# trifectatechfoundation/zlib-rs

Hardware: NVIDIA H100
Metric: deflate_level6_raw_input_throughput_silesia_small_tar (higher is better)
Workload: dtype u8

## Files before the change

zlib_rs_b200/csrc/zb_engine.cu:

```cuda
#include <cuda_runtime.h>
#include <stdio.h>
#include <stdlib.h>
#include <string.h>
#include <new>
#include "../../include/zb_engine.h"
#include "zb_kernels.cuh"
#include "zb_engine_internal.h"

namespace zb {

constexpr uint32_t kSlowSub9 = 24576;
constexpr uint32_t kTailTiles = 2;
constexpr uint32_t kTailSub = 512;

thread_local char g_err[256] = "";

static void set_err(const char *what, cudaError_t e)
{
    snprintf(g_err, sizeof g_err, "%s: %s", what, cudaGetErrorString(e));
}

#define CK(call)                                                  \
    do {                                                          \
        cudaError_t e_ = (call);                                  \
        if (e_ != cudaSuccess) { set_err(#call, e_); return ZB_E_CUDA; } \
    } while (0)

__global__ void k_match(JobBufs);
__global__ void k_skip(JobBufs);
__global__ void k_nxt(JobBufs);
__global__ void k_path_tiles(JobBufs);
__global__ void k_path_chain(JobBufs, uint32_t, uint32_t);
__global__ void k_path_groups(JobBufs, uint32_t, uint32_t, uint4 *, uint32_t *);
__global__ void k_path_chain2(JobBufs, uint32_t, uint32_t, const uint4 *, uint32_t *, uint32_t *);
__global__ void k_path_mark(JobBufs, const uint32_t *, const uint32_t *);
__global__ void k_iter_lists(JobBufs, uint32_t *, uint32_t *, uint32_t);
__global__ void k_emit(JobBufs);
__global__ void k_holes(JobBufs, uint32_t);
__global__ void k_holes_cmp(JobBufs, uint32_t, uint32_t);
__global__ void k_tail(JobBufs);
__global__ void k_block_hist(JobBufs, uint32_t *);
__global__ void k_build_blocks(JobBufs, const uint32_t *);
__global__ void k_scan_blocks(JobBufs);
__global__ void k_encode(JobBufs);
__global__ void k_finish(JobBufs, const uint32_t *);
__global__ void k_literal_syms(JobBufs);
__global__ void k_stored(JobBufs);
__global__ void k_links2_std(JobBufs, uint32_t);
__global__ void k_links2_roll(JobBufs, uint32_t);
__global__ void k_links_fix_std(JobBufs);
__global__ void k_links_fix_roll(JobBufs);
__global__ void k_slow(JobBufs);
__global__ void k_rle(JobBufs);
__global__ void k_emit_slow(JobBufs);
__global__ void k_tail_slow(JobBufs);
__global__ void k_serial_low(JobBufs);
__global__ void k_links_dict_ghost(JobBufs, uint32_t *);
__global__ void k_links_dict_ghost_apply(JobBufs, const uint32_t *);
__global__ void k_bgzf_setup(BgzfJob, uint64_t);
__global__ void k_serial_low_members(JobBufs, BgzfJob);
__global__ void k_bgzf_medium(JobBufs, BgzfJob);
__global__ void k_bgzf_slow_steps(JobBufs, BgzfJob);
__global__ void k_bgzf_slow_walk(JobBufs, BgzfJob);
__global__ void k_bgzf_hist(JobBufs, BgzfJob, uint32_t *);
__global__ void k_bgzf_build(JobBufs, BgzfJob, const uint32_t *);
__global__ void k_bgzf_size(JobBufs, BgzfJob);
__global__ void k_bgzf_scan(JobBufs, BgzfJob);
__global__ void k_bgzf_encode(JobBufs, BgzfJob);
__global__ void k_bgzf_frame(JobBufs, BgzfJob);

constexpr uint32_t kMatchSmemBytes = (kWSize + kMatchSub + 512) + (kWSize + kMatchSub) * 2 + ((kWSize + kMatchSub) / 32 + 1) * 4 * 4 + 8192;
constexpr uint32_t kPathSmemBytes = kPathTile * 4 * 3;
constexpr uint32_t kLinks2SmemBytes = 65536 * 2 + kLinkTile * 2 + kLinkTile + 64 + 2048;
constexpr uint32_t kSkipSmemBytes = 2 * kWSize * 2 + 2 * (2 * kWSize / 32) * 4 + 8192 + 64;
constexpr uint32_t kSlowSubMax = 24576;
constexpr uint32_t kSlowSmemBytes = (kWSize + kSlowSubMax + kSlowAhead) * 3;
constexpr uint32_t kChainSmemBytes = kChainChunkTiles * kPathHead * 8;
constexpr uint32_t kChain2MaxSmem = 200 * 1024;
constexpr uint32_t kSerialSmemBytes = (65536 + kWSize) * 2 + 35824 + 16;
constexpr uint32_t kSerialSmemQuick = 65536 * 2 + 65536 + 16;

int Engine::init(int dev)
{
    int n = 0;
    cudaError_t e = cudaGetDeviceCount(&n);
    if (e != cudaSuccess || n == 0) {
        snprintf(g_err, sizeof g_err, "no CUDA device (%s)", e == cudaSuccess ? "count 0" : cudaGetErrorString(e));
        return ZB_E_NODEVICE;
    }
    if (dev < 0 || dev >= n) { snprintf(g_err, sizeof g_err, "device %d out of range", dev); return ZB_E_PARAM; }
    device = dev;
    CK(cudaSetDevice(dev));
    CK(cudaStreamCreateWithFlags(&st, cudaStreamNonBlocking));
    CK(cudaStreamCreateWithFlags(&st2, cudaStreamNonBlocking));
    CK(cudaEventCreateWithFlags(&evf, cudaEventDisableTiming));
    CK(cudaEventCreateWithFlags(&evt, cudaEventDisableTiming));
    for (int i = 0; i < kUpChunks; i++) CK(cudaEventCreateWithFlags(&evc[i], cudaEventDisableTiming));
    CK(cudaEventCreateWithFlags(&evk, cudaEventDisableTiming));
    CK(cudaEventCreate(&ev0));
    CK(cudaEventCreate(&ev1));
    CK(upload_tables());
    CK(cudaFuncSetAttribute(k_match, cudaFuncAttributeMaxDynamicSharedMemorySize, kMatchSmemBytes));
    CK(cudaFuncSetAttribute(k_skip, cudaFuncAttributeMaxDynamicSharedMemorySize, kSkipSmemBytes));
    CK(cudaFuncSetAttribute(k_links2_std, cudaFuncAttributeMaxDynamicSharedMemorySize, kLinks2SmemBytes));
    CK(cudaFuncSetAttribute(k_links2_roll, cudaFuncAttributeMaxDynamicSharedMemorySize, kLinks2SmemBytes));
    CK(cudaFuncSetAttribute(k_slow, cudaFuncAttributeMaxDynamicSharedMemorySize, kSlowSmemBytes));
    CK(cudaFuncSetAttribute(k_path_tiles, cudaFuncAttributeMaxDynamicSharedMemorySize, kPathSmemBytes));
    CK(cudaFuncSetAttribute(k_path_mark, cudaFuncAttributeMaxDynamicSharedMemorySize, kPathSmemBytes));
    CK(cudaFuncSetAttribute(k_path_chain, cudaFuncAttributeMaxDynamicSharedMemorySize, kChainSmemBytes));
    CK(cudaFuncSetAttribute(k_path_groups, cudaFuncAttributeMaxDynamicSharedMemorySize, kChain2MaxSmem));
    CK(cudaFuncSetAttribute(k_path_chain2, cudaFuncAttributeMaxDynamicSharedMemorySize, kChain2MaxSmem));
    CK(cudaFuncSetAttribute(k_serial_low, cudaFuncAttributeMaxDynamicSharedMemorySize, kSerialSmemBytes));
    CK(cudaFuncSetAttribute(k_serial_low_members, cudaFuncAttributeMaxDynamicSharedMemorySize, kSerialSmemBytes));
    CK(cudaMallocHost(&h_info, sizeof(JobInfo)));
    CK(cudaMalloc(&d_info, sizeof(JobInfo)));
    CK(cudaMalloc(&d_check, 16));
    { int rc_ = inflate_init(); if (rc_ != ZB_OK) return rc_; }
    return ZB_OK;
}

Engine::~Engine()
{
    if (device < 0) return;
    cudaSetDevice(device);
    for (auto &b : bufs) if (b.p) cudaFree(b.p);
    if (h_stage) cudaFreeHost(h_stage);
    if (h_info) cudaFreeHost(h_info);
    if (d_info) cudaFree(d_info);
    if (d_check) cudaFree(d_check);
    if (ev0) cudaEventDestroy(ev0);
    if (ev1) cudaEventDestroy(ev1);
    if (evf) cudaEventDestroy(evf);
    if (evt) cudaEventDestroy(evt);
    for (int i = 0; i < kUpChunks; i++) if (evc[i]) cudaEventDestroy(evc[i]);
    if (evk) cudaEventDestroy(evk);
    if (st2) cudaStreamDestroy(st2);
    if (st) cudaStreamDestroy(st);
}

void Engine::pbegin()
{
    if (!profile) return;
    if (!pev0) { cudaEventCreate(&pev0); cudaEventCreate(&pev1); }
    cudaEventRecord(pev0, st);
}

void Engine::pend(int phase, uint32_t nlaunch)
{
    if (!profile) return;
    cudaEventRecord(pev1, st);
    cudaEventSynchronize(pev1);
    float ms = 0;
    cudaEventElapsedTime(&ms, pev0, pev1);
    phase_ms[phase] += ms;
    phase_launches[phase] += nlaunch;
}

int Engine::reserve(int slot, size_t bytes, void **out)
{
    Buf &b = bufs[slot];
    if (b.cap < bytes) {
        if (b.p) { cudaFree(b.p); b.p = nullptr; b.cap = 0; }
        size_t want = bytes + (bytes >> 3) + 4096;
        cudaError_t e = cudaMalloc(&b.p, want);
        if (e != cudaSuccess) { set_err("cudaMalloc", e); return ZB_E_MEM; }
        b.cap = want;
// ... 229 lines not shown
        pend(9, 0);
    }
    CK(cudaMemsetAsync(d_info, 0, sizeof(JobInfo), st));
    CK(cudaMemsetAsync(d_out, 0, out_cap, st));
    if (jb.prime_bits) {
        h_prime = (uint8_t)((flags >> 16) & ((1u << jb.prime_bits) - 1u));
        CK(cudaMemcpyAsync(d_out, &h_prime, 1, cudaMemcpyHostToDevice, st));
    }
    cudaStream_t st_ck = chunked_upload ? st2 : st;
    pbegin();
    if (wrap == 1 || (wrap == 0 && (flags & ZB_FLAG_CHECK_ADLER))) { CK(launch_adler32(d_in + dstart, n_in, 1, d_ck, ck_bytes, d_check, st_ck)); launches += 2; }
    else if (wrap == 2 || (wrap == 0 && (flags & ZB_FLAG_CHECK_CRC))) { CK(launch_crc32(d_in + dstart, n_in, 0, d_ck, ck_bytes, d_check, st_ck)); launches += 2; }
    else CK(cudaMemsetAsync(d_check, 0, 4, st_ck));
    if (chunked_upload) CK(cudaEventRecord(evk, st2));
    pend(8, 2);

    auto links_tiles = [&](bool roll) {
        uint32_t t_done = 0;
        for (uint32_t k = 0; k < (chunked_upload ? up_chunks : 1u); k++) {
            uint32_t t_hi = nmt;
            if (chunked_upload) {
                cudaStreamWaitEvent(st, evc[k], 0);
                if (k + 1 < up_chunks) t_hi = up_len[k] >= 64 ? (uint32_t)((up_len[k] - 64) / kLinkTile) : 0;
            }
            if (t_hi <= t_done) continue;
            if (roll) k_links2_roll<<<t_hi - t_done, 1024, kLinks2SmemBytes, st>>>(jb, t_done);
            else k_links2_std<<<t_hi - t_done, 1024, kLinks2SmemBytes, st>>>(jb, t_done);
            if (k) launches++;
            t_done = t_hi;
        }
        if (chunked_upload) cudaStreamWaitEvent(st, evk, 0);
    };
    uint32_t iters = 0;
    if (level == 0) {
        const uint32_t nb = n_in == 0 ? 1 : (uint32_t)((n_in + 65534) / 65535);
        k_stored<<<nb, 256, 0, st>>>(jb);
        launches++;
        k_finish<<<1, 32, 0, st>>>(jb, d_check);
        launches++;
    } else {
        if (jb.huffman_only) {
            k_literal_syms<<<(uint32_t)(n_in / 256 + 1), 256, 0, st>>>(jb);
            launches++;
        } else if (jb.serial_mode) {
            iters = 1;
            pbegin();
            k_serial_low<<<1, 32, jb.serial_mode == 2 ? kSerialSmemBytes : kSerialSmemQuick, st>>>(jb);
            launches++;
            pend(1, 1);
        } else {
            CK(cudaMemsetAsync(jb.holes, 0, (size_t)nwords * 4, st));
            CK(cudaMemsetAsync(jb.holes_new, 0, (size_t)nwords * 4, st));
            CK(cudaMemsetAsync(jb.tile_dirty, 1, nmt, st));
            CK(cudaMemsetAsync(jb.tile_entry, 0xee, (size_t)npt * 4, st));
            CK(cudaMemsetAsync(jb.M + N, 0, (size_t)kPad * 4, st));
            CK(cudaMemsetAsync(jb.L + N, 0, (size_t)kPad * 2, st));
            pbegin();
            if (jb.slow_mode == 2) {
            } else if (jb.slow_mode && jb.sp.slow) {
                links_tiles(true);
                k_links_fix_roll<<<N / 256 + 1, 256, 0, st>>>(jb);
                launches += 2;
            } else {
                links_tiles(false);
                k_links_fix_std<<<N / 256 + 1, 256, 0, st>>>(jb);
                launches += 2;
// ... 74 lines not shown
                    pbegin();
                    k_path_tiles<<<n_ptiles, 1024, kPathSmemBytes, st>>>(jb);
                    launch_chain(first_ptile);
                    launch_mark(iters == 1 ? npt : 2 * n_ptiles + 16);
                    pend(3, 3);
                    pbegin();
                    k_holes<<<(nlists * kLongPerSub + 255) / 256, 256, 0, st>>>(jb, nlists);
                    k_holes_cmp<<<(nwords + 255) / 256, 256, 0, st>>>(jb, nwords, nmt);
                    pend(4, 2);
                    launches += 7;
                    k_iter_lists<<<1, 1024, 0, st>>>(jb, d_lists, d_lists + nmt + 8, npt);
                    launches++;
                    CK(cudaMemcpyAsync(h_info, d_info, sizeof(JobInfo), cudaMemcpyDeviceToHost, st));
                    CK(cudaStreamSynchronize(st));
                    if (h_info->error) { snprintf(g_err, sizeof g_err, "engine error flags 0x%x (parse)", h_info->error); return ZB_E_INTERNAL; }
                    if (getenv("ZB_DEBUG")) {
                        static unsigned long long last[3];
                        if (iters == 1) memset(last, 0, sizeof last);
                        const double ctas = (double)(h_info->dbg[0] - last[0]) + 1e-9;
                        fprintf(stderr, "iter %u dirty %u: ctas %llu stage %.1f walk %.1f kcyc/cta, holes_changed %u, sub %u first_tile %u chain %u\n",
                                iters, n_dirty, h_info->dbg[0] - last[0], (h_info->dbg[1] - last[1]) / 1e3 / ctas,
                                (h_info->dbg[2] - last[2]) / 1e3 / ctas, h_info->holes_changed, jb.match_sub, first_ptile, chain2 ? 2u : 1u);
                        memcpy(last, h_info->dbg, sizeof last);
                    }
                    if (!h_info->holes_changed) break;
                    n_dirty = h_info->n_dirty;
                    if (iters > N / 257u + 4096u) { snprintf(g_err, sizeof g_err, "hole iteration did not converge"); return ZB_E_INTERNAL; }
                }
            }
            CK(cudaEventRecord(evf, st));
            CK(cudaStreamWaitEvent(st2, evf, 0));
            k_tail<<<1, 32, 0, st2>>>(jb);
            launches++;
            CK(cudaEventRecord(evt, st2));
            if (jb.tail_start > 0) {
                pbegin();
                k_emit<<<(jb.tail_start + 255) / 256, 256, 0, st>>>(jb);
                launches++;
                pend(4, 1);
            }
            pbegin();
            CK(cudaStreamWaitEvent(st, evt, 0));
            pend(5, 1);
            }
        }
        CK(cudaMemcpyAsync(h_info, d_info, sizeof(JobInfo), cudaMemcpyDeviceToHost, st));
        CK(cudaStreamSynchronize(st));
        if (h_info->error) { snprintf(g_err, sizeof g_err, "engine error flags 0x%x (tail)", h_info->error); return ZB_E_INTERNAL; }
        const uint32_t nblocks = h_info->n_blocks;
        if (nblocks == 0 || nblocks > max_blocks) { snprintf(g_err, sizeof g_err, "bad block count %u", nblocks); return ZB_E_INTERNAL; }
        pbegin();
        k_block_hist<<<nblocks, 256, 0, st>>>(jb, d_freq);
        k_build_blocks<<<nblocks, 32, 0, st>>>(jb, d_freq);
        k_scan_blocks<<<1, 256, 0, st>>>(jb);
        pend(6, 3);
        pbegin();
        k_encode<<<nblocks, 1024, 0, st>>>(jb);
        k_finish<<<1, 32, 0, st>>>(jb, d_check);
        pend(7, 2);
        launches += 5;
    }
    CK(cudaMemcpyAsync(h_info, d_info, sizeof(JobInfo), cudaMemcpyDeviceToHost, st));
    CK(cudaStreamSynchronize(st));
    CK(cudaGetLastError());
    if (h_info->error) {
        if (h_info->error & 8u) return ZB_E_BUF;
        snprintf(g_err, sizeof g_err, "engine error flags 0x%x (encode)", h_info->error);
        return ZB_E_INTERNAL;
    }
    const uint64_t out_bytes = h_info->out_bytes;
    if (out_bytes > dst_cap) {
        res->out_bytes = out_bytes;
        return ZB_E_BUF;
    }
    if (d_out != dst) {
        pbegin();
        CK(cudaMemcpyAsync(dst, d_out, out_bytes, dst_dev ? cudaMemcpyDeviceToDevice : cudaMemcpyDeviceToHost, st));
        pend(10, 0);
    }
    CK(cudaEventRecord(ev1, st));
    CK(cudaStreamSynchronize(st));
    float ms = 0;
    CK(cudaEventElapsedTime(&ms, ev0, ev1));
    res->out_bytes = out_bytes;
    res->check = h_info->adler;
    res->data_type = (int32_t)h_info->data_type;
    res->iterations = iters;
    res->n_symbols = h_info->n_syms;
    res->n_blocks = h_info->n_blocks;
    res->gpu_launches = launches;
    res->exact_parity = exact ? 1 : 0;
    res->gpu_ms = ms;
    res->bits_used = (uint32_t)(h_info->total_bits & 7u) ? (uint32_t)(h_info->total_bits & 7u) : 8u;
// ... 337 lines not shown
```

zlib_rs_b200/csrc/zb_engine_internal.h:

```cpp
#pragma once
#include <cuda_runtime.h>
#include <stddef.h>
#include <stdint.h>
#include "../../include/zb_engine.h"
#include "zb_kernels.cuh"

namespace zb {

extern thread_local char g_err[256];
size_t deflate_bound(size_t n);

enum { S_IN, S_L, S_HOLES, S_HOLESN, S_M, S_NXT, S_PEXIT, S_PCNT, S_SYMIDX, S_TENTRY, S_TSYMB, S_TDIRTY, S_SYMS, S_SYMB,
       S_BLOCKS, S_SCRATCH, S_FREQ, S_OUT, S_CK, S_INF0, S_INF1, S_PHEAD, S_SK, S_MARKN, S_LLIST, S_LCNT, S_BMAP, S_HDIFF, S_HCOARSE, S_CSTATE, S_LISTS, S_LR, S_LLAST, S_BBASE, S_MCHG, S_GFN, S_KEYS, S_SHARD,
       S_MEMT, S_MEMC,
       S_BGZF,
       S_COUNT };

struct ShardState {
    int phase = 0;
    JobBufs jb;
    uint32_t off = 0, S = 0, E = 0, total = 0;
    uint32_t bs = 0, npt = 0, O = 0, n = 0, blo = 0, nloc = 0;
    bool is_last = false, tables = false;
    uint4 *gfn = nullptr;
    uint32_t chainG = 0, chain_groups = 0, chain2_smem = 0;
    uint32_t freq_lo[320], freq_hi[320];
    zb_shard_span span;
};

struct Engine {
    static constexpr int kSlots = 41;
    struct Buf { void *p = nullptr; size_t cap = 0; };
    int device = -1;
    cudaStream_t st = nullptr, st2 = nullptr;
    cudaEvent_t evf = nullptr, evt = nullptr;
    cudaEvent_t ev0 = nullptr, ev1 = nullptr;
    static constexpr int kUpChunks = 8;
    cudaEvent_t evk = nullptr;
    cudaEvent_t evc[kUpChunks] = {nullptr};
    Buf bufs[kSlots];
    void *h_stage = nullptr;
    size_t h_stage_cap = 0;
    JobInfo *h_info = nullptr, *d_info = nullptr;
    uint32_t *d_check = nullptr;
    void *d_inf_state = nullptr, *h_inf_state = nullptr;
    uint32_t launches = 0;
    uint8_t h_prime = 0;
    static constexpr int kPhases = 12;
    bool profile = false;
    float phase_ms[kPhases] = {0};
    uint32_t phase_launches[kPhases] = {0};
    cudaEvent_t pev0 = nullptr, pev1 = nullptr;
    void pbegin();
    void pend(int phase, uint32_t nlaunch);

    int init(int dev);
    int inflate_init();
    ~Engine();
    int reserve(int slot, size_t bytes, void **out);
    int stage(size_t bytes);
    int deflate(const void *src, size_t n, bool src_dev, void *dst, size_t dst_cap, bool dst_dev, int level, int strategy,
                int window_bits, uint32_t flags, zb_deflate_result *res, const void *dict = nullptr, size_t dict_len = 0);
    int deflate_bgzf(const void *src, size_t n, bool src_dev, void *dst, size_t dst_cap, bool dst_dev, int level, zb_deflate_result *res);
    int inflate(const void *src, size_t n, bool src_dev, void *dst, size_t dst_cap, bool dst_dev, int window_bits,
                zb_inflate_result *res, uint32_t flags = 0);
    int inflate_stream(const uint8_t *d_src, size_t n, uint8_t *d_dst, size_t dst_cap, int window_bits, uint32_t flags,
                       zb_inflate_result *res);
    int inflate_members(const uint8_t *d_src, size_t n, uint8_t *d_dst, size_t dst_cap, int window_bits, zb_inflate_result *res);
// ... 15 lines not shown
```

zlib_rs_b200/csrc/zb_kernels.cu:

```cuda
#include "zb_kernels.cuh"

namespace zb {

__constant__ HuffTables c_tab;

cudaError_t upload_tables()
{
    HuffTables t;
    init_tables(t);
    return cudaMemcpyToSymbol(c_tab, &t, sizeof t);
}

struct GAcc {
    const uint8_t *data;
    uint32_t N;
    const uint16_t *L;
    const uint32_t *holes;
    const uint32_t *M;
    uint32_t w = kWSize;
    __device__ __forceinline__ uint32_t byte(uint32_t y) const
    {
        while (y >= N) {
            if (y < 2 * w) return 0;
            y -= w;
// ... 1112 lines not shown
        syms[k] = s;
        sb[k] = B;
        k++;
    };
    uint32_t fb;
    if (jb.wsize == kWSize) fb = serial_medium(a, jb.N, p0, ins, 1024u, jb.lp, emit);
    else fb = serial_medium(GAccW{a, jb.wsize}, jb.N, p0, ins, 1024u, jb.lp, emit, DynWin{jb.wsize});
    jb.info->n_syms = n_mid + k;
    jb.info->final_base = fb;
    jb.info->n_blocks = (n_mid + k) / jb.block_syms + 1;
}

__device__ __forceinline__ uint32_t sym_end(const Sym &s) { return s.pos + (s.dist ? (uint32_t)s.lc + 3u : 1u); }

__device__ __forceinline__ void block_hist_body(const Sym *syms, uint32_t begin, uint32_t count, uint32_t *fb)
{
    __shared__ uint32_t lf[kLCodes], df[kDCodes];
    for (uint32_t i = threadIdx.x; i < kLCodes; i += blockDim.x) lf[i] = 0;
    if (threadIdx.x < kDCodes) df[threadIdx.x] = 0;
    __syncthreads();
    for (uint32_t i = threadIdx.x; i < count; i += blockDim.x) {
        const Sym s = syms[begin + i];
        if (s.dist == 0) atomicAdd(&lf[s.lc], 1u);
        else {
            atomicAdd(&lf[257 + c_tab.length_code[s.lc]], 1u);
            atomicAdd(&df[d_code(c_tab, s.dist - 1u)], 1u);
        }
    }
    __syncthreads();
    for (uint32_t i = threadIdx.x; i < kLCodes; i += blockDim.x) fb[i] = lf[i];
    if (threadIdx.x < kDCodes) fb[kLCodes + threadIdx.x] = df[threadIdx.x];
}

__global__ void __launch_bounds__(256) k_block_hist(JobBufs jb, uint32_t *freq )
{
    const uint32_t b = blockIdx.x;
    const uint32_t nsyms = jb.info->n_syms, nblocks = jb.info->n_blocks;
    const uint32_t begin = b * jb.block_syms;
    const uint32_t count = (b + 1 < nblocks) ? jb.block_syms : nsyms - begin;
    block_hist_body(jb.syms, begin, count, freq + b * 320);
    if (threadIdx.x == 0) {
        BlockDesc &bd = jb.blocks[b];
        const bool last = b + 1 == nblocks;
        bd.sym_begin = begin;
        bd.sym_count = count;
        bd.last = last && !jb.not_last;
        const uint32_t start = begin == 0 ? jb.start : sym_end(jb.syms[begin - 1]);
        const uint32_t end = last ? jb.N : sym_end(jb.syms[begin + count - 1]);
        bd.in_start = start;
        bd.in_len = end - start;
        uint32_t Bf;
        if (last) Bf = jb.info->final_base;
        else {
            const uint32_t li = begin + count - 1, n_mid = jb.info->n_mid_syms;
            if (jb.serial_mode) {
                Bf = jb.serial_mode == 2 ? jb.block_base[b] : 0;
            } else if (jb.huffman_only) {
                const uint32_t q = jb.syms[li].pos, w = jb.wsize;
                Bf = q < 2 * w ? 0 : w * (1 + (q - 2 * w) / w);
            } else if (jb.slow_mode == 2) {
                Bf = base_at(jb.syms[li].pos, jb.N, jb.wsize);
            } else if (jb.slow_mode) {
                Bf = base_at(jb.syms[li].pos + 1, jb.N, jb.wsize);
            } else Bf = li < n_mid ? wbase_w(DynWin{jb.wsize}, jb.syms[li].pos) : jb.sym_base[li - n_mid];
        }
        bd.have_window = start >= Bf;
    }
}

__device__ __forceinline__ uint32_t brev_bits(uint32_t code, uint32_t len) { return __brev(code) >> (32u - len); }

template <int KIND>
__device__ __forceinline__ uint32_t xbits_of(uint32_t n) { return KIND == 0 ? (n >= 257 ? extra_lbits(n - 257) : 0u) : KIND == 1 ? extra_dbits(n) : extra_blbits(n); }

template <int KIND>
__device__ int build_tree_warp(TreeScratch &s, TreeState &st, CtData *tree, uint32_t *sh_cnt )
{
    constexpr int elems = KIND == 0 ? kLCodes : KIND == 1 ? kDCodes : kBlCodes;
    constexpr int max_length = KIND == 2 ? kMaxBlBits : kMaxBits;
    const uint32_t lane = threadIdx.x & 31;
    int heap_len = 0, max_code = -1;
    for (int b0 = 0; b0 < elems; b0 += 32) {
        const int n = b0 + (int)lane;
        const bool nz = n < elems && tree[n].fc != 0;
        const uint32_t m = __ballot_sync(0xffffffffu, nz);
        if (nz) { s.heap[heap_len + 1 + __popc(m & ((1u << lane) - 1u))] = (uint32_t)n; s.depth[n] = 0; }
        else if (n < elems) tree[n].dl = 0;
        heap_len += __popc(m);
        if (m) max_code = b0 + 31 - __clz(m);
    }
    __syncwarp();
    if (heap_len < 2) {
        if (lane == 0) {
            while (heap_len < 2) {
                const int node = max_code < 2 ? ++max_code : 0;
                s.heap[++heap_len] = (uint32_t)node;
                tree[node].fc = 1;
// ... 217 lines not shown
            o.put((uint32_t)(blcodes - 4), 4);
            for (int r = 0; r < blcodes; r++) o.put(s.bltree[bl_order(r)].dl, 3);
            send_tree_fast(o, s.bltree, s.ltree, lcodes - 1);
            send_tree_fast(o, s.bltree, s.dtree, dcodes - 1);
            b.hdr_bits = o.nbits;
            b.body_bits = 3 + st.opt_len - o.nbits;
        }
        for (int n = (int)lane; n < kLCodes; n += 32) { b.lcode[n] = n <= lmax ? s.ltree[n].fc : 0; b.llen[n] = n <= lmax ? (uint8_t)s.ltree[n].dl : 0; }
        if (lane < (uint32_t)kDCodes) { b.dcode[lane] = (int)lane <= dmax ? s.dtree[lane].fc : 0; b.dlen[lane] = (int)lane <= dmax ? (uint8_t)s.dtree[lane].dl : 0; }
    }
    __syncwarp();
}

__device__ __forceinline__ void build_blocks_body(BlockDesc *gbd, const uint32_t *fb, bool quick, bool first, bool last_piece,
                                                  bool final_block, bool strategy_fixed)
{
    __shared__ TreeScratch s;
    __shared__ BlockDesc bd;
    __shared__ uint32_t fr[320];
    __shared__ uint32_t sh_cnt[16];
    __shared__ TreeState sh_st;
    for (uint32_t i = threadIdx.x; i < 320; i += 32) fr[i] = fb[i];
    for (uint32_t i = threadIdx.x; i < sizeof(BlockDesc) / 4; i += 32)
        reinterpret_cast<uint32_t *>(&bd)[i] = reinterpret_cast<const uint32_t *>(gbd)[i];
    __syncwarp();
    if (quick) {
        if (threadIdx.x == 0) build_quick_piece(c_tab, bd, fr, fr + kLCodes, first, last_piece, final_block);
    } else build_block_warp(s, bd, fr, fr + kLCodes, bd.have_window != 0, strategy_fixed, sh_cnt, &sh_st);
    __syncwarp();
    for (uint32_t i = threadIdx.x; i < sizeof(BlockDesc) / 4; i += 32)
        reinterpret_cast<uint32_t *>(gbd)[i] = reinterpret_cast<const uint32_t *>(&bd)[i];
}

__global__ void __launch_bounds__(32) k_build_blocks(JobBufs jb, const uint32_t *freq)
{
    const uint32_t b = blockIdx.x;
    if (b >= jb.info->n_blocks) return;
    build_blocks_body(&jb.blocks[b], freq + b * 320, jb.serial_mode == 1, b == 0, b + 1 == jb.info->n_blocks, jb.not_last == 0,
                      jb.strategy_fixed != 0);
}

__device__ __forceinline__ void or_bits(uint32_t *out32, uint64_t pos, uint64_t val, uint32_t n)
{
    if (n == 0) return;
    const uint64_t w = pos >> 5;
    const uint32_t sh = (uint32_t)(pos & 31);
    atomicOr(&out32[w], (uint32_t)(val << sh));
    if (sh + n > 32) {
        atomicOr(&out32[w + 1], (uint32_t)(val >> (32 - sh)));
        if (sh + n > 64) atomicOr(&out32[w + 2], (uint32_t)(val >> (64 - sh)));
    }
}

constexpr uint32_t kScanChunk = 1024;
__global__ void __launch_bounds__(256) k_scan_blocks(JobBufs jb)
{
    __shared__ uint64_t s_bits[kScanChunk];
    __shared__ uint64_t s_base[kScanChunk];
    __shared__ uint64_t s_bit;
    const uint32_t nb = jb.info->n_blocks;
    if (threadIdx.x == 0) s_bit = 8ull * jb.hdr_len + jb.prime_bits;
    for (uint32_t c0 = 0; c0 < nb; c0 += kScanChunk) {
        const uint32_t nc = min(kScanChunk, nb - c0);
        for (uint32_t i = threadIdx.x; i < nc; i += blockDim.x) {
            const BlockDesc &bd = jb.blocks[c0 + i];
            s_bits[i] = bd.type == 0 ? (1ull << 63) | (uint16_t)bd.in_len : (uint64_t)bd.hdr_bits + bd.body_bits;
        }
        __syncthreads();
        if (threadIdx.x == 0) {
            uint64_t bit = s_bit;
            for (uint32_t i = 0; i < nc; i++) {
                s_base[i] = bit;
                const uint64_t v = s_bits[i];
                bit = (v >> 63) ? ((bit + 3 + 7) & ~7ull) + 32 + 8ull * (v & 0xffffu) : bit + v;
            }
            s_bit = bit;
        }
        __syncthreads();
        for (uint32_t i = threadIdx.x; i < nc; i += blockDim.x) jb.blocks[c0 + i].bit_base = s_base[i];
        __syncthreads();
    }
    if (threadIdx.x != 0) return;
    uint64_t bit = s_bit;
    if (jb.not_last && jb.end_mode == 0) {
        const uint64_t p = (bit + 3 + 7) & ~7ull;
        jb.info->marker_byte = p >> 3;
        bit = p + 32;
    } else if (jb.not_last && jb.end_mode == 1) {
        or_bits(reinterpret_cast<uint32_t *>(jb.out), bit, 2u, 10);
        bit += 10;
    }
    jb.info->total_bits = bit;
    const uint64_t bytes = (jb.not_last && jb.end_mode ? (bit >> 3) : ((bit + 7) >> 3)) + (jb.wrap == 1 ? 4 : jb.wrap == 2 ? 8 : 0);
    jb.info->out_bytes = bytes;
    jb.info->data_type = jb.blocks[0].sym_count ? jb.blocks[0].data_type : 2u;
    if (bytes > jb.out_cap) { atomicOr(&jb.info->error, 8u); return; }
    if (jb.wrap == 1) {
        const uint32_t lf = (jb.huffman_only || jb.strategy_fixed || jb.level < 2) ? 0 : jb.level < 6 ? 1 : jb.level == 6 ? 2 : 3;
        uint32_t h = ((8u + (jb.cinfo << 4)) << 8) | (lf << 6);
        h += 31 - (h % 31);
        jb.out[0] = (uint8_t)(h >> 8);
        jb.out[1] = (uint8_t)h;
    } else if (jb.wrap == 2) {
        const uint8_t g[10] = {31, 139, 8, 0, 0, 0, 0, 0, (uint8_t)jb.xfl, 3};
        for (int i = 0; i < 10; i++) jb.out[i] = g[i];
    }
}

__device__ __forceinline__ void encode_body(const BlockDesc &bd, const Sym *syms, const uint8_t *in, uint8_t *out, uint32_t *error)
{
    __shared__ HuffTables st;
    __shared__ uint16_t s_lcode[kLCodes], s_dcode[kDCodes];
    __shared__ uint8_t s_llen[kLCodes], s_dlen[kDCodes];
    __shared__ uint64_t warp_sum[32];
    uint32_t *out32 = reinterpret_cast<uint32_t *>(out);
// ... 58 lines not shown
            lens[j] = (uint8_t)n;
            mybits += n;
        }
        uint64_t incl = mybits;
#pragma unroll
        for (int o = 1; o < 32; o <<= 1) {
            const uint64_t t = __shfl_up_sync(0xffffffffu, incl, o);
            if ((int)lane >= o) incl += t;
        }
        if (lane == 31) warp_sum[warp] = incl;
        __syncthreads();
        if (warp == 0) {
            uint64_t ws = warp_sum[lane];
#pragma unroll
            for (int o = 1; o < 32; o <<= 1) {
                const uint64_t t = __shfl_up_sync(0xffffffffu, ws, o);
                if ((int)lane >= o) ws += t;
            }
            warp_sum[lane] = ws;
        }
        __syncthreads();
        uint64_t pos = bd.bit_base + bd.hdr_bits + round_bits + (incl - mybits) + (warp ? warp_sum[warp - 1] : 0);
#pragma unroll
        for (uint32_t j = 0; j < kSymsPerThread; j++) {
            or_bits(out32, pos, vals[j], lens[j]);
            pos += lens[j];
        }
        round_bits += warp_sum[31];
        __syncthreads();
    }
    if (tid == blockDim.x - 1 && round_bits != bd.body_bits) atomicOr(error, 16u);
}

__global__ void __launch_bounds__(1024) k_encode(JobBufs jb)
{
    if (jb.info->error) return;
    encode_body(jb.blocks[blockIdx.x], jb.syms, jb.in, jb.out, &jb.info->error);
}

__global__ void __launch_bounds__(256) k_bgzf_hist(JobBufs jb, BgzfJob bj, uint32_t *freq)
{
    const uint32_t b = blockIdx.x, m = b / kBgzfMaxBlocks, k = b % kBgzfMaxBlocks;
    const JobInfo &mi = bj.minfo[m];
    const uint32_t nsyms = mi.n_syms, nblocks = mi.n_blocks;
    if (k >= nblocks) return;
    const uint32_t base = m * kBgzfStride, len = bj.mlen[m];
    const Sym *syms = jb.syms + base;
    const uint32_t begin = k * jb.block_syms;
    const uint32_t count = k + 1 < nblocks ? jb.block_syms : nsyms - begin;
    block_hist_body(syms, begin, count, freq + (size_t)b * 320);
    if (threadIdx.x == 0) {
        BlockDesc &bd = jb.blocks[b];
        const bool last = k + 1 == nblocks;
        bd.sym_begin = base + begin;
        bd.sym_count = count;
        bd.last = last;
        const uint32_t start = begin == 0 ? 0 : sym_end(syms[begin - 1]);
        const uint32_t end = last ? len : sym_end(syms[begin + count - 1]);
        bd.in_start = base + start;
        bd.in_len = end - start;
        uint32_t Bf;
        if (last) Bf = mi.final_base;
        else if (jb.slow_mode) Bf = base_at(syms[begin + count - 1].pos + 1, len, jb.wsize);
        else Bf = jb.block_base[b];
        bd.have_window = start >= Bf;
    }
}

__global__ void __launch_bounds__(32) k_bgzf_build(JobBufs jb, BgzfJob bj, const uint32_t *freq)
{
// ... 106 lines not shown
```

zlib_rs_b200/csrc/zb_shard.cu:

```cuda
#include <stdio.h>
#include <string.h>
#include "zb_kernels.cuh"
#include "zb_engine_internal.h"
#include "zb_shard.h"

namespace zb {

__global__ void k_slow(JobBufs);
__global__ void k_links2_std(JobBufs, uint32_t);
__global__ void k_links2_roll(JobBufs, uint32_t);
__global__ void k_links_fix_std(JobBufs);
__global__ void k_links_fix_roll(JobBufs);
__global__ void k_path_tiles(JobBufs);
__global__ void k_path_chain(JobBufs, uint32_t, uint32_t);
__global__ void k_path_groups(JobBufs, uint32_t, uint32_t, uint4 *, uint32_t *);
__global__ void k_path_chain2(JobBufs, uint32_t, uint32_t, const uint4 *, uint32_t *, uint32_t *);
__global__ void k_path_mark(JobBufs, const uint32_t *, const uint32_t *);
__global__ void k_emit_slow(JobBufs);
__global__ void k_tail_slow(JobBufs);
__global__ void k_build_blocks(JobBufs, const uint32_t *);
__global__ void k_scan_blocks(JobBufs);
__global__ void k_encode(JobBufs);

static __constant__ HuffTables s_tab;

constexpr uint32_t kLinks2Smem = 65536 * 2 + kLinkTile * 2 + kLinkTile + 64 + 2048;
constexpr uint32_t kPathSmem = kPathTile * 4 * 3;
constexpr uint32_t kChainSmem = kChainChunkTiles * kPathHead * 8;
constexpr uint32_t kChain2Max = 200 * 1024;

__global__ void __launch_bounds__(128) k_shard_entry(JobBufs jb, uint32_t S, uint32_t E, uint2 *out)
{
    const uint32_t c = blockIdx.x * blockDim.x + threadIdx.x;
    if (c >= kShardCand) return;
    const uint32_t te = jb.info->tail_entry;
    uint32_t spec_total = jb.info->n_mid_syms, spec_exit = te;
    if (te < E) { const uint32_t v = jb.nxt[te]; spec_total += (v >> 16) & 0xffu; spec_exit = te + (v & 0xffffu); }
    uint32_t p = S + c, cnt = 0, steps = 0;
    while (p < E) {
        const uint32_t idx = jb.symidx[p];
        if (idx) {
            const uint32_t k = jb.tile_symbase[p / kPathTile] + idx - 1;
            out[c] = make_uint2(spec_exit, cnt + spec_total - k);
            return;
        }
        const uint32_t v = jb.nxt[p];
        if ((v & 0xffffu) == 0 || ++steps > E) { atomicOr(&jb.info->error, 1u); return; }
        cnt += (v >> 16) & 0xffu;
        p += v & 0xffffu;
    }
    out[c] = make_uint2(p, cnt);
}

__global__ void __launch_bounds__(256) k_shard_hist(JobBufs jb, uint32_t *freq, ShardLoc *loc, uint32_t O, uint32_t n, uint32_t blo,
                                                    uint32_t bs)
// ... 286 lines not shown
    if (nl > shard.nloc) {
        const ShardLoc e{ns, 0, 0, 0, 0, 0, {0, 0}};
        SCK(cudaMemcpyAsync(d_loc + shard.nloc, &e, sizeof e, cudaMemcpyHostToDevice, st));
        SCK(cudaMemsetAsync(d_freq + (size_t)shard.nloc * 320, 0, 320 * 4, st));
        if (shard.nloc) memset(shard.freq_hi, 0, sizeof shard.freq_hi);
        else { memset(shard.freq_lo, 0, sizeof shard.freq_lo); memset(shard.freq_hi, 0, sizeof shard.freq_hi); }
        shard.nloc = nl;
        shard.blo = lo;
    }
    const uint32_t nloc = shard.nloc;
    if (!nloc) { shard.phase = 3; shard.span = *span; return ZB_OK; }
    uint32_t holds = 0;
    static thread_local BlockDesc hb;
    static thread_local ShardBlock m;
    for (int k = 0; k < 2; k++) {
        const uint32_t j = k == 0 ? 0 : nloc - 1, b = shard.blo + j;
        if (shard_merge(all, n, pl, b, bs, shard.total, m) != 0) return shard_param("edge records do not add up");
        SCK(cudaMemcpyAsync(&hb, jb.blocks + j, sizeof hb, cudaMemcpyDeviceToHost, st));
        SCK(cudaStreamSynchronize(st));
        hb.sym_count = m.nsyms;
        hb.in_start = m.in_start >= off ? m.in_start - off : 0u;
        hb.in_len = m.in_end - m.in_start;
        hb.last = b == pl.fin;
        hb.have_window = m.in_start >= m.flush_base;
        SCK(cudaMemcpyAsync(jb.blocks + j, &hb, sizeof hb, cudaMemcpyHostToDevice, st));
        SCK(cudaMemcpyAsync(d_freq + (size_t)j * 320, m.freq, 320 * 4, cudaMemcpyHostToDevice, st));
        SCK(cudaStreamSynchronize(st));
        holds |= (shard_holds_first(O, ns, shard.is_last, pl, b, bs) ? 1u : 0u) << (2 * k);
        holds |= (shard_holds_last(O, ns, shard.is_last, pl, b, bs) ? 2u : 0u) << (2 * k);
    }
    SCK(cudaMemcpyAsync(d_xloc, shard.freq_lo, 320 * 4, cudaMemcpyHostToDevice, st));
    SCK(cudaMemcpyAsync(d_xloc + 320, shard.freq_hi, 320 * 4, cudaMemcpyHostToDevice, st));
    SCK(cudaMemcpyAsync(&d_info->n_blocks, &nloc, 4, cudaMemcpyHostToDevice, st));
    k_build_blocks<<<nloc, 32, 0, st>>>(jb, d_freq);
    k_shard_piece<<<1, 256, 0, st>>>(jb, d_freq, d_xloc, d_loc, nloc, holds, d_span);
    SCK(cudaMemcpyAsync(span, d_span, sizeof *span, cudaMemcpyDeviceToHost, st));
    SCK(cudaMemcpyAsync(h_info, d_info, sizeof(JobInfo), cudaMemcpyDeviceToHost, st));
    SCK(cudaStreamSynchronize(st));
    SCK(cudaGetLastError());
    if (h_info->error) { snprintf(g_err, sizeof g_err, "engine error flags 0x%x (shard size)", h_info->error); return ZB_E_INTERNAL; }
    shard.span = *span;
    shard.phase = 3;
    return ZB_OK;
}

int Engine::shard_encode(uint64_t bit_offset, void *dst, size_t cap, bool dst_dev, uint64_t *bytes)
{
    if (shard.phase != 3) { shard.phase = 0; return shard_param("zb_shard_encode needs zb_shard_size first"); }
    if (!bytes) { shard.phase = 0; return shard_param("null argument"); }
    JobBufs &jb = shard.jb;
    const uint32_t prime = (uint32_t)(bit_offset & 7u);
    const uint64_t end = shard_span_end(shard.span, prime), need = (end + 7) >> 3;
    *bytes = need;
    if (cap < need || (!dst && need)) return ZB_E_BUF;
    shard.phase = 0;
    if (!need) return ZB_OK;
    SCK(cudaSetDevice(device));
    if (!shard.nloc) {
        if (dst_dev) SCK(cudaMemset(dst, 0, need)); else memset(dst, 0, need);
        return ZB_OK;
    }
    void *p;
    int rc;
    const size_t out_cap = (need + 64) & ~(size_t)15;
    if ((rc = reserve(S_OUT, out_cap + 16, &p)) != ZB_OK) return rc;
    jb.out = static_cast<uint8_t *>(p);
    jb.out_cap = out_cap;
    jb.prime_bits = prime;
    jb.wrap = 0;
    jb.hdr_len = 0;
    jb.not_last = 0;
    SCK(cudaMemsetAsync(jb.out, 0, out_cap, st));
    k_scan_blocks<<<1, 256, 0, st>>>(jb);
    k_encode<<<shard.nloc, 1024, 0, st>>>(jb);
    SCK(cudaMemcpyAsync(h_info, d_info, sizeof(JobInfo), cudaMemcpyDeviceToHost, st));
    SCK(cudaStreamSynchronize(st));
    SCK(cudaGetLastError());
    if (h_info->error || h_info->total_bits != end) {
        snprintf(g_err, sizeof g_err, "engine error flags 0x%x, %llu bits for a span of %llu (shard encode)", h_info->error,
                 (unsigned long long)h_info->total_bits, (unsigned long long)end);
        return ZB_E_INTERNAL;
    }
    SCK(cudaMemcpyAsync(dst, jb.out, need, dst_dev ? cudaMemcpyDeviceToDevice : cudaMemcpyDeviceToHost, st));
    SCK(cudaStreamSynchronize(st));
    return ZB_OK;
}

}

extern "C" {

struct zb_engine { zb::Engine e; };

int zb_shard_parse(zb_engine *z, const void *src, size_t total_len, int src_on_device, size_t range_begin, size_t range_end, int level,
                   int strategy, uint32_t flags, zb_shard_entry *table, uint32_t *adler)
{
    if (!z) return ZB_E_NODEVICE;
    return z->e.shard_parse(src, total_len, src_on_device != 0, range_begin, range_end, level, strategy, flags, table, adler);
}

int zb_shard_symbols(zb_engine *z, uint32_t entry, uint32_t sym_offset, zb_shard_edge *first, zb_shard_edge *last)
{
    if (!z) return ZB_E_NODEVICE;
    return z->e.shard_symbols(entry, sym_offset, first, last);
}

int zb_shard_size(zb_engine *z, const zb_shard_edge *all, size_t n, zb_shard_span *span)
// ... 13 lines not shown
```

Measured before the change: 1.596.

## Overlap path-block histogram, build and encode with the serial tail stream

Splits block histogram, build, scan and encode into a path-derived prefix of blocks and a tail-derived remainder. The prefix blocks are built and encoded on the main stream while k_tail runs on the second stream, and the tail blocks are histogrammed there too. This also drops the host round-trip that read back the block count before encoding, using an over-sized grid with in-kernel bounds checks instead. In exchange the grid size is estimated on the host, with a device error flag raised if it is too small, and the kernel signatures and scan logic become more complex.

```diff
diff --git a/zlib_rs_b200/csrc/zb_engine.cu b/zlib_rs_b200/csrc/zb_engine.cu
--- a/zlib_rs_b200/csrc/zb_engine.cu
+++ b/zlib_rs_b200/csrc/zb_engine.cu
@@ -39,10 +39,10 @@
 __global__ void k_holes(JobBufs, uint32_t);
 __global__ void k_holes_cmp(JobBufs, uint32_t, uint32_t);
 __global__ void k_tail(JobBufs);
-__global__ void k_block_hist(JobBufs, uint32_t *);
-__global__ void k_build_blocks(JobBufs, const uint32_t *);
-__global__ void k_scan_blocks(JobBufs);
-__global__ void k_encode(JobBufs);
+__global__ void k_block_hist(JobBufs, uint32_t *, uint32_t, uint32_t);
+__global__ void k_build_blocks(JobBufs, const uint32_t *, uint32_t, uint32_t);
+__global__ void k_scan_blocks(JobBufs, uint32_t, uint32_t);
+__global__ void k_encode(JobBufs, uint32_t, uint32_t);
 __global__ void k_finish(JobBufs, const uint32_t *);
 __global__ void k_literal_syms(JobBufs);
 __global__ void k_stored(JobBufs);
@@ -95,6 +95,7 @@
     CK(cudaStreamCreateWithFlags(&st2, cudaStreamNonBlocking));
     CK(cudaEventCreateWithFlags(&evf, cudaEventDisableTiming));
     CK(cudaEventCreateWithFlags(&evt, cudaEventDisableTiming));
+    CK(cudaEventCreateWithFlags(&evp, cudaEventDisableTiming));
     for (int i = 0; i < kUpChunks; i++) CK(cudaEventCreateWithFlags(&evc[i], cudaEventDisableTiming));
     CK(cudaEventCreateWithFlags(&evk, cudaEventDisableTiming));
     CK(cudaEventCreate(&ev0));
@@ -132,6 +133,7 @@
     if (ev1) cudaEventDestroy(ev1);
     if (evf) cudaEventDestroy(evf);
     if (evt) cudaEventDestroy(evt);
+    if (evp) cudaEventDestroy(evp);
     for (int i = 0; i < kUpChunks; i++) if (evc[i]) cudaEventDestroy(evc[i]);
     if (evk) cudaEventDestroy(evk);
     if (st2) cudaStreamDestroy(st2);
@@ -427,6 +429,7 @@
         if (chunked_upload) cudaStreamWaitEvent(st, evk, 0);
     };
     uint32_t iters = 0;
+    uint32_t path_blocks = 0, tail_grid = 0;
     if (level == 0) {
         const uint32_t nb = n_in == 0 ? 1 : (uint32_t)((n_in + 65534) / 65535);
         k_stored<<<nb, 256, 0, st>>>(jb);
@@ -567,33 +570,60 @@
             CK(cudaStreamWaitEvent(st2, evf, 0));
             k_tail<<<1, 32, 0, st2>>>(jb);
             launches++;
-            CK(cudaEventRecord(evt, st2));
+            path_blocks = jb.tail_start > 0 ? h_info->n_mid_syms / block_syms : 0u;
+            if (path_blocks) {
+                const uint32_t p0 = h_info->tail_entry > jb.start ? h_info->tail_entry : jb.start;
+                tail_grid = (uint32_t)(((uint64_t)h_info->n_mid_syms + (N - p0)) / block_syms) + 1u - path_blocks;
+            }
             if (jb.tail_start > 0) {
                 pbegin();
                 k_emit<<<(jb.tail_start + 255) / 256, 256, 0, st>>>(jb);
                 launches++;
                 pend(4, 1);
             }
+            if (path_blocks) {
+                CK(cudaEventRecord(evp, st));
+                CK(cudaStreamWaitEvent(st2, evp, 0));
+                k_block_hist<<<tail_grid, 256, 0, st2>>>(jb, d_freq, path_blocks, 0);
+                k_build_blocks<<<tail_grid, 32, 0, st2>>>(jb, d_freq, path_blocks, 0);
+                pbegin();
+                k_block_hist<<<path_blocks, 256, 0, st>>>(jb, d_freq, 0, 1);
+                k_build_blocks<<<path_blocks, 32, 0, st>>>(jb, d_freq, 0, 1);
+                k_scan_blocks<<<1, 256, 0, st>>>(jb, 0, path_blocks);
+                k_encode<<<path_blocks, 1024, 0, st>>>(jb, 0, 0);
+                pend(6, 4);
+                launches += 6;
+            }
+            CK(cudaEventRecord(evt, st2));
             pbegin();
             CK(cudaStreamWaitEvent(st, evt, 0));
             pend(5, 1);
             }
         }
-        CK(cudaMemcpyAsync(h_info, d_info, sizeof(JobInfo), cudaMemcpyDeviceToHost, st));
-        CK(cudaStreamSynchronize(st));
-        if (h_info->error) { snprintf(g_err, sizeof g_err, "engine error flags 0x%x (tail)", h_info->error); return ZB_E_INTERNAL; }
-        const uint32_t nblocks = h_info->n_blocks;
-        if (nblocks == 0 || nblocks > max_blocks) { snprintf(g_err, sizeof g_err, "bad block count %u", nblocks); return ZB_E_INTERNAL; }
-        pbegin();
-        k_block_hist<<<nblocks, 256, 0, st>>>(jb, d_freq);
-        k_build_blocks<<<nblocks, 32, 0, st>>>(jb, d_freq);
-        k_scan_blocks<<<1, 256, 0, st>>>(jb);
-        pend(6, 3);
-        pbegin();
-        k_encode<<<nblocks, 1024, 0, st>>>(jb);
-        k_finish<<<1, 32, 0, st>>>(jb, d_check);
-        pend(7, 2);
-        launches += 5;
+        if (path_blocks) {
+            pbegin();
+            k_scan_blocks<<<1, 256, 0, st>>>(jb, path_blocks, 0xffffffffu);
+            k_encode<<<tail_grid, 1024, 0, st>>>(jb, path_blocks, 1);
+            k_finish<<<1, 32, 0, st>>>(jb, d_check);
+            pend(7, 3);
+            launches += 3;
+        } else {
+            CK(cudaMemcpyAsync(h_info, d_info, sizeof(JobInfo), cudaMemcpyDeviceToHost, st));
+            CK(cudaStreamSynchronize(st));
+            if (h_info->error) { snprintf(g_err, sizeof g_err, "engine error flags 0x%x (tail)", h_info->error); return ZB_E_INTERNAL; }
+            const uint32_t nblocks = h_info->n_blocks;
+            if (nblocks == 0 || nblocks > max_blocks) { snprintf(g_err, sizeof g_err, "bad block count %u", nblocks); return ZB_E_INTERNAL; }
+            pbegin();
+            k_block_hist<<<nblocks, 256, 0, st>>>(jb, d_freq, 0, 0);
+            k_build_blocks<<<nblocks, 32, 0, st>>>(jb, d_freq, 0, 0);
+            k_scan_blocks<<<1, 256, 0, st>>>(jb, 0, 0xffffffffu);
+            pend(6, 3);
+            pbegin();
+            k_encode<<<nblocks, 1024, 0, st>>>(jb, 0, 0);
+            k_finish<<<1, 32, 0, st>>>(jb, d_check);
+            pend(7, 2);
+            launches += 5;
+        }
     }
     CK(cudaMemcpyAsync(h_info, d_info, sizeof(JobInfo), cudaMemcpyDeviceToHost, st));
     CK(cudaStreamSynchronize(st));
diff --git a/zlib_rs_b200/csrc/zb_engine_internal.h b/zlib_rs_b200/csrc/zb_engine_internal.h
--- a/zlib_rs_b200/csrc/zb_engine_internal.h
+++ b/zlib_rs_b200/csrc/zb_engine_internal.h
@@ -34,6 +34,7 @@
     int device = -1;
     cudaStream_t st = nullptr, st2 = nullptr;
     cudaEvent_t evf = nullptr, evt = nullptr;
+    cudaEvent_t evp = nullptr;
     cudaEvent_t ev0 = nullptr, ev1 = nullptr;
     static constexpr int kUpChunks = 8;
     cudaEvent_t evk = nullptr;
diff --git a/zlib_rs_b200/csrc/zb_kernels.cu b/zlib_rs_b200/csrc/zb_kernels.cu
--- a/zlib_rs_b200/csrc/zb_kernels.cu
+++ b/zlib_rs_b200/csrc/zb_kernels.cu
@@ -1168,10 +1168,12 @@
     if (threadIdx.x < kDCodes) fb[kLCodes + threadIdx.x] = df[threadIdx.x];
 }
 
-__global__ void __launch_bounds__(256) k_block_hist(JobBufs jb, uint32_t *freq )
-{
-    const uint32_t b = blockIdx.x;
-    const uint32_t nsyms = jb.info->n_syms, nblocks = jb.info->n_blocks;
+__global__ void __launch_bounds__(256) k_block_hist(JobBufs jb, uint32_t *freq , uint32_t b0, uint32_t path_only)
+{
+    const uint32_t b = b0 + blockIdx.x;
+    const uint32_t nsyms = path_only ? 0u : jb.info->n_syms, nblocks = path_only ? 0xffffffffu : jb.info->n_blocks;
+    if (!path_only && threadIdx.x == 0 && blockIdx.x == 0 && nblocks > b0 + gridDim.x) atomicOr(&jb.info->error, 256u);
+    if (b >= nblocks) return;
     const uint32_t begin = b * jb.block_syms;
     const uint32_t count = (b + 1 < nblocks) ? jb.block_syms : nsyms - begin;
     block_hist_body(jb.syms, begin, count, freq + b * 320);
@@ -1198,7 +1200,7 @@
                 Bf = base_at(jb.syms[li].pos, jb.N, jb.wsize);
             } else if (jb.slow_mode) {
                 Bf = base_at(jb.syms[li].pos + 1, jb.N, jb.wsize);
-            } else Bf = li < n_mid ? wbase_w(DynWin{jb.wsize}, jb.syms[li].pos) : jb.sym_base[li - n_mid];
+            } else Bf = path_only || li < n_mid ? wbase_w(DynWin{jb.wsize}, jb.syms[li].pos) : jb.sym_base[li - n_mid];
         }
         bd.have_window = start >= Bf;
     }
@@ -1482,11 +1484,12 @@
         reinterpret_cast<uint32_t *>(gbd)[i] = reinterpret_cast<const uint32_t *>(&bd)[i];
 }
 
-__global__ void __launch_bounds__(32) k_build_blocks(JobBufs jb, const uint32_t *freq)
-{
-    const uint32_t b = blockIdx.x;
-    if (b >= jb.info->n_blocks) return;
-    build_blocks_body(&jb.blocks[b], freq + b * 320, jb.serial_mode == 1, b == 0, b + 1 == jb.info->n_blocks, jb.not_last == 0,
+__global__ void __launch_bounds__(32) k_build_blocks(JobBufs jb, const uint32_t *freq, uint32_t b0, uint32_t path_only)
+{
+    const uint32_t b = b0 + blockIdx.x;
+    const uint32_t nblocks = path_only ? 0xffffffffu : jb.info->n_blocks;
+    if (b >= nblocks) return;
+    build_blocks_body(&jb.blocks[b], freq + b * 320, jb.serial_mode == 1, b == 0, b + 1 == nblocks, jb.not_last == 0,
                       jb.strategy_fixed != 0);
 }
 
@@ -1503,26 +1506,26 @@
 }
 
 constexpr uint32_t kScanChunk = 1024;
-__global__ void __launch_bounds__(256) k_scan_blocks(JobBufs jb)
+__device__ __forceinline__ uint64_t block_bits(const BlockDesc &bd) { return bd.type == 0 ? (1ull << 63) | (uint16_t)bd.in_len : (uint64_t)bd.hdr_bits + bd.body_bits; }
+__device__ __forceinline__ uint64_t block_end_bit(uint64_t bit, uint64_t v) { return (v >> 63) ? ((bit + 3 + 7) & ~7ull) + 32 + 8ull * (v & 0xffffu) : bit + v; }
+
+__global__ void __launch_bounds__(256) k_scan_blocks(JobBufs jb, uint32_t b0, uint32_t b1)
 {
     __shared__ uint64_t s_bits[kScanChunk];
     __shared__ uint64_t s_base[kScanChunk];
     __shared__ uint64_t s_bit;
-    const uint32_t nb = jb.info->n_blocks;
-    if (threadIdx.x == 0) s_bit = 8ull * jb.hdr_len + jb.prime_bits;
-    for (uint32_t c0 = 0; c0 < nb; c0 += kScanChunk) {
+    const bool to_end = b1 == 0xffffffffu;
+    const uint32_t nb = to_end ? jb.info->n_blocks : b1;
+    if (threadIdx.x == 0) s_bit = b0 ? block_end_bit(jb.blocks[b0 - 1].bit_base, block_bits(jb.blocks[b0 - 1])) : 8ull * jb.hdr_len + jb.prime_bits;
+    for (uint32_t c0 = b0; c0 < nb; c0 += kScanChunk) {
         const uint32_t nc = min(kScanChunk, nb - c0);
-        for (uint32_t i = threadIdx.x; i < nc; i += blockDim.x) {
-            const BlockDesc &bd = jb.blocks[c0 + i];
-            s_bits[i] = bd.type == 0 ? (1ull << 63) | (uint16_t)bd.in_len : (uint64_t)bd.hdr_bits + bd.body_bits;
-        }
+        for (uint32_t i = threadIdx.x; i < nc; i += blockDim.x) s_bits[i] = block_bits(jb.blocks[c0 + i]);
         __syncthreads();
         if (threadIdx.x == 0) {
             uint64_t bit = s_bit;
             for (uint32_t i = 0; i < nc; i++) {
                 s_base[i] = bit;
-                const uint64_t v = s_bits[i];
-                bit = (v >> 63) ? ((bit + 3 + 7) & ~7ull) + 32 + 8ull * (v & 0xffffu) : bit + v;
+                bit = block_end_bit(bit, s_bits[i]);
             }
             s_bit = bit;
         }
@@ -1530,7 +1533,7 @@
         for (uint32_t i = threadIdx.x; i < nc; i += blockDim.x) jb.blocks[c0 + i].bit_base = s_base[i];
         __syncthreads();
     }
-    if (threadIdx.x != 0) return;
+    if (threadIdx.x != 0 || !to_end) return;
     uint64_t bit = s_bit;
     if (jb.not_last && jb.end_mode == 0) {
         const uint64_t p = (bit + 3 + 7) & ~7ull;
@@ -1655,10 +1658,11 @@
     if (tid == blockDim.x - 1 && round_bits != bd.body_bits) atomicOr(error, 16u);
 }
 
-__global__ void __launch_bounds__(1024) k_encode(JobBufs jb)
+__global__ void __launch_bounds__(1024) k_encode(JobBufs jb, uint32_t b0, uint32_t to_end)
 {
     if (jb.info->error) return;
-    encode_body(jb.blocks[blockIdx.x], jb.syms, jb.in, jb.out, &jb.info->error);
+    if (to_end && b0 + blockIdx.x >= jb.info->n_blocks) return;
+    encode_body(jb.blocks[b0 + blockIdx.x], jb.syms, jb.in, jb.out, &jb.info->error);
 }
 
 __global__ void __launch_bounds__(256) k_bgzf_hist(JobBufs jb, BgzfJob bj, uint32_t *freq)
diff --git a/zlib_rs_b200/csrc/zb_shard.cu b/zlib_rs_b200/csrc/zb_shard.cu
--- a/zlib_rs_b200/csrc/zb_shard.cu
+++ b/zlib_rs_b200/csrc/zb_shard.cu
@@ -18,9 +18,9 @@
 __global__ void k_path_mark(JobBufs, const uint32_t *, const uint32_t *);
 __global__ void k_emit_slow(JobBufs);
 __global__ void k_tail_slow(JobBufs);
-__global__ void k_build_blocks(JobBufs, const uint32_t *);
-__global__ void k_scan_blocks(JobBufs);
-__global__ void k_encode(JobBufs);
+__global__ void k_build_blocks(JobBufs, const uint32_t *, uint32_t, uint32_t);
+__global__ void k_scan_blocks(JobBufs, uint32_t, uint32_t);
+__global__ void k_encode(JobBufs, uint32_t, uint32_t);
 
 static __constant__ HuffTables s_tab;
 
@@ -373,7 +373,7 @@
     SCK(cudaMemcpyAsync(d_xloc, shard.freq_lo, 320 * 4, cudaMemcpyHostToDevice, st));
     SCK(cudaMemcpyAsync(d_xloc + 320, shard.freq_hi, 320 * 4, cudaMemcpyHostToDevice, st));
     SCK(cudaMemcpyAsync(&d_info->n_blocks, &nloc, 4, cudaMemcpyHostToDevice, st));
-    k_build_blocks<<<nloc, 32, 0, st>>>(jb, d_freq);
+    k_build_blocks<<<nloc, 32, 0, st>>>(jb, d_freq, 0, 0);
     k_shard_piece<<<1, 256, 0, st>>>(jb, d_freq, d_xloc, d_loc, nloc, holds, d_span);
     SCK(cudaMemcpyAsync(span, d_span, sizeof *span, cudaMemcpyDeviceToHost, st));
     SCK(cudaMemcpyAsync(h_info, d_info, sizeof(JobInfo), cudaMemcpyDeviceToHost, st));
@@ -412,8 +412,8 @@
     jb.hdr_len = 0;
     jb.not_last = 0;
     SCK(cudaMemsetAsync(jb.out, 0, out_cap, st));
-    k_scan_blocks<<<1, 256, 0, st>>>(jb);
-    k_encode<<<shard.nloc, 1024, 0, st>>>(jb);
+    k_scan_blocks<<<1, 256, 0, st>>>(jb, 0, 0xffffffffu);
+    k_encode<<<shard.nloc, 1024, 0, st>>>(jb, 0, 0);
     SCK(cudaMemcpyAsync(h_info, d_info, sizeof(JobInfo), cudaMemcpyDeviceToHost, st));
     SCK(cudaStreamSynchronize(st));
     SCK(cudaGetLastError());
```

After: 1.622 (median of 6 runs). 1.02x the previous value.
